# url-kaist/UV-SLAM

Measured on AMD Instinct MI355X. Metric: sliding-window solves/sec (10 KF, 150 pts, 40 lines, 3 VP), higher is better.
Workload: dtype f64; 1 GPU; W10-P150-L40-V3 x 256 independent windows per GPU (BASELINE configs[2]); single window (configs[1]) in single_window, the 20k-point window (configs[3]) in large_window (both with --full); windows_per_gpu=256, frames=11, points=150, lines=40, vp_tagged_lines=30, prior=True, parallelism=replicas x1

## Files before the change

uv-slam_amd/api.py:

```python
import ctypes as C
import os
import time

import numpy as np

from . import abi

_HERE = os.path.dirname(os.path.abspath(__file__))
LIB_PATH = os.environ.get("UVS_SOLVER_LIB", os.path.join(_HERE, "libuvs_solver.so"))
_lib = None

EXPORTS = [
    "uvs_abi_version", "uvs_default_options", "uvs_create", "uvs_destroy", "uvs_last_error", "uvs_status_string",
    "uvs_solve_window", "uvs_batch_upload", "uvs_batch_solve", "uvs_batch_download", "uvs_batch_stream", "uvs_evaluate", "uvs_marginalize", "uvs_marginalize_resident", "uvs_marginalize_batch",
    "uvs_reduced_dim", "uvs_pg_create", "uvs_pg_destroy", "uvs_pg_last_error", "uvs_pg_optimize", "uvs_pg_debug_step",
    "uvs_lc_create", "uvs_lc_destroy", "uvs_lc_last_error", "uvs_lc_verify", "uvs_lc_debug_pair",
    "uvs_vp_create", "uvs_vp_destroy", "uvs_vp_last_error", "uvs_vp_estimate", "uvs_vp_last_device_ms", "uvs_vp_debug_frame",
    "uvs_kf_create", "uvs_kf_destroy", "uvs_kf_last_error", "uvs_kf_extract", "uvs_kf_last_device_ms", "uvs_kf_debug_frame",
    "uvs_ft_create", "uvs_ft_destroy", "uvs_ft_last_error", "uvs_ft_reset", "uvs_ft_track", "uvs_ft_last_device_ms", "uvs_ft_debug_pyramid", "uvs_ft_debug_point",
    "uvs_ft_set_max_candidates", "uvs_ft_set_mask", "uvs_ft_detect", "uvs_ft_last_detect_device_ms", "uvs_ft_debug_detect",
    "uvs_ft_reject", "uvs_ft_last_reject_device_ms", "uvs_ft_debug_reject",
    "uvs_ft_set_equalize", "uvs_ft_equalize", "uvs_ft_last_equalize_device_ms", "uvs_ft_debug_equalize",
    "uvs_lt_create", "uvs_lt_destroy", "uvs_lt_last_error", "uvs_lt_reset", "uvs_lt_track", "uvs_lt_match", "uvs_lt_last_device_ms", "uvs_lt_debug_line",
    "uvs_lt_gauss_tables",
# ... 453 lines not shown
        try:
            for s, rc in zip(solvers, rcs): s._check(rc)

            def exchange(which, n):
                bufs = [np.zeros(n) for _ in solvers]
                for s, b in zip(solvers, bufs): s._check(L.uvs_large_exchange_host(s._h, which, abi._dp(b), 0))
                tot = bufs[0].copy()
                for b in bufs[1:]: tot = tot + b
                if which == 0: tot[n - 7] = max(b[n - 7] for b in bufs)
                for s in solvers: s._check(L.uvs_large_exchange_host(s._h, which, abi._dp(tot), 1))

            n = C.c_int(0)
            L.uvs_large_reduced(solvers[0]._h, C.byref(n)); n_red = n.value
            L.uvs_large_scalars(solvers[0]._h, C.byref(n)); n_sc = n.value
            for k in range(len(r)):
                for s in solvers:
                    assert L.uvs_large_need_linearize(s._h)
                    s._check(L.uvs_large_linearize(s._h))
                exchange(0, n_red)
                for s in solvers: s._check(L.uvs_large_step(s._h))
                exchange(1, n_sc)
                for s, (step, scal) in zip(solvers, out):
                    s._check(L.uvs_large_debug_step(s._h, float(r[k + 1]) if k + 1 < len(r) else 0.0, step.shape[1], abi._dp(step[k]), abi._dp(scal[k])))
        finally:
            for s in solvers:
                L.uvs_large_set_debug_step(s._h, 0); L.uvs_large_set_nranks(s._h, 1)
        return out

    def debug_first_iteration(self, w: abi.Window):
        wc, keep = w.to_c()
        S = np.zeros((176, 176)); g = np.zeros(176); hd = np.zeros(176); dd = np.zeros(176); step = np.zeros(176); scal = np.zeros(40)
        self._check(lib().uvs_debug_first_iteration(self._h, C.byref(wc), *[abi._dp(a) for a in (S, g, hd, dd, step, scal)]))
        return dict(S=S, g=g, hd=hd, dd=dd, step=step, cost=scal[0], gmax=scal[1], chol_ok=scal[2], mcc=scal[3], step2=scal[4],
                    cycles=dict(zip(['setup', 'obs', 'lmprep', 'gather', 'assemble', 'chol', 'trsv', 'backsub', 'cost', 'misc', 'chol_diag', 'chol_panel', 'chol_trail', 'asm_imu', 'asm_zero', 'asm_add'], scal[8:24])), sub_timers=dict(cost_phase=dict(zip(['stage_dx', 'prior_residual', 'observations', 'imu'], scal[24:28])), chol_busy_per_wave=scal[28:32].copy()))


class PoseGraphSolver(_Handle):

    _UNIT = "uvs_pg"

    def __init__(self, device=0, max_keyframes=16384, max_loops=256):
        self._create(device, max_keyframes, max_loops)

    def optimize_raw(self, t, q, sequence, constant, loops):
        p, keep = abi.pg_problem(t, q, sequence, constant, loops)
        out = np.zeros((max(p.n, 1), 4))
        rep = abi.PgReport()
        t0 = time.perf_counter()
        rc = lib().uvs_pg_optimize(self._h, C.byref(p), abi._dp(out), C.byref(rep))
        self.last_ms = (time.perf_counter() - t0) * 1e3
        return rc, out[:p.n], rep

    def optimize(self, t, q, sequence, constant, loops):
        rc, out, rep = self.optimize_raw(t, q, sequence, constant, loops)
        if rc not in (abi.UVS_OK, abi.UVS_ERR_NUMERIC):
            raise self._error("uvs_pg_optimize", rc)
        return out, rep

    def debug_step_raw(self, t, q, sequence, constant, loops, radius):
        p, keep = abi.pg_problem(t, q, sequence, constant, loops)
        delta = np.zeros(max(4 * int(np.count_nonzero(keep["constant"] == 0)), 1)); scal = np.zeros(abi.PG_DEBUG_SCAL_LEN)
        rc = lib().uvs_pg_debug_step(self._h, C.byref(p), float(radius), abi._dp(delta), abi._dp(scal))
        return rc, delta[:4 * int(scal[3])], scal

    def debug_step(self, t, q, sequence, constant, loops, radius):
        rc, delta, scal = self.debug_step_raw(t, q, sequence, constant, loops, radius)
# ... 886 lines not shown
```

uv-slam_amd/csrc/uvs_layout.h:

```cpp
#pragma once
#include <stdint.h>

#define UVS_NF 11
#define UVS_FD 16
#define UVS_RD (UVS_NF * UVS_FD)
#define UVS_NBLK (UVS_NF * (UVS_NF + 1) / 2)
#define UVS_NBLKX (UVS_NBLK + UVS_NF + 1 + UVS_NF + 2)
#define UVS_EX_INDEX(a) (16 * (a) + 15)
#define UVS_RELO_FRAME (UVS_NF + 1)
#define UVS_RELO2_BLOCKROW (UVS_NF + 2)
#define UVS_NBLKX2 (UVS_NBLKX + UVS_NF + 3)
#define UVS_RELO2_DOUBLES 2304
#define UVS_XDIM 192
#define UVS_TD_INDEX (UVS_RD - 1)
#define UVS_BLK_LD 17
#define UVS_BLK_SZ (16 * UVS_BLK_LD)
#define UVS_S_DOUBLES (UVS_NBLK * UVS_BLK_SZ)

#define UVS_IMU_STRIDE 296
#define UVS_IMU_JAC 20
#define UVS_IMU_COV 68
#define UVS_IMU_WS 226
#define UVS_IMU_JIDX(R, C, i, j) (9 * ((R) == 0 ? ((C) == 9 ? 0 : 1) : (R) == 3 ? 2 : ((C) == 9 ? 3 : 4)) + 3 * (i) + (j))

// ... 52 lines not shown
    int32_t d_lnmeas;
    int32_t d_imu;
    int32_t d_prior;
    int32_t i_pt_lm, i_pt_fi, i_pt_fj, i_pt_beg;
    int32_t i_ln_lm, i_ln_fj, i_ln_vp, i_ln_beg;
    int32_t i_imu;
    int32_t i_prior;
    int32_t i_chunks;
    int32_t i_wblk;
    int32_t i_lists;
    int32_t w_invd0, w_invd1, w_line0, w_line1;
    int32_t w_ltrig0, w_ltrig1;
    int32_t w_scale_pt, w_scale_ln;
    int32_t w_pt_E, w_pt_x;
    int32_t w_ln_Y, w_ln_x;
    int32_t w_imu;
    int32_t w_imu_w;
    int32_t w_out;
    int32_t w_prior_h0;
    int32_t n_pblk;
    int32_t w_gacc;
    int32_t n_cimg, w_cimg;
    int32_t ws_doubles;
    int32_t blob_bytes;
    int32_t cur_sel;
    int32_t max_chunk_doubles;
    int32_t n_parts;
    int32_t chol_half_ok;
    int32_t reserved0;
    int64_t out_host;
    int32_t redamp_ok;
};

#define UVS_PH_G0(n) ((((n) * (n)) + 1) & ~1)
#define UVS_PH_C0(n) (UVS_PH_G0(n) + UVS_MAX_PRIOR_DIM)
#define UVS_PH_HD(n) (UVS_PH_C0(n) + 8)
#define UVS_PH_DOUBLES(n) (UVS_PH_HD(n) + UVS_RD)
#define UVS_WIMU_STRIDE 936
#define UVS_LN_X 24
```

uv-slam_amd/csrc/uvs_solve_kernel.h:

```cpp
#pragma once
#include <hip/hip_runtime.h>
#include <initializer_list>
#include <utility>
#include "../../include/uvs_solver.h"
#include "uvs_layout.h"
#include "uvs_factors.h"

namespace uvsdev {

#ifndef UVS_UNIT
#define UVS_UNIT unit
#endif

#ifndef UVS_X_PLAIN_TID
static __device__ __forceinline__ int lane_tid() { int t = threadIdx.x; asm volatile("" : "+v"(t)); return t; }
#else
static __device__ __forceinline__ int lane_tid() { return threadIdx.x; }
#endif
static constexpr int NT = UVS_NT;
static constexpr int NW = NT / 64;
static constexpr bool ROLES = NT > 256;
static constexpr int ET = ROLES ? 256 : NT;
static constexpr int EW = ET / 64;
static constexpr int GT0 = NT - UVS_GT;
// ... 33 lines not shown
static constexpr int L_PRC = L_PR + UVS_MAX_PRIOR_DIM;
static constexpr int L_RED = L_PRC + UVS_MAX_PRIOR_DIM;
static constexpr int L_CTRL = L_RED + (5 * NW > 24 ? 5 * NW : 24);
static constexpr int L_PROF = L_CTRL + 32;
static constexpr int L_WPROF = L_PROF + 24;
static constexpr int L_LCOST = L_WPROF + 8;
static constexpr int LACC = 1;
static constexpr int L_LGMAX = L_LCOST + ET / LACC;
static constexpr int L_PX0 = L_LGMAX + 8;
static constexpr int L_PTAB = L_PX0 + 9 * UVS_MAX_PRIOR_BLOCKS;
static constexpr int L_SMALL = (L_PTAB + 2 * UVS_MAX_PRIOR_BLOCKS + 1) & ~1;
static constexpr int L_S = L_SMALL;
static constexpr int L_TOTAL = L_S + UVS_S_DOUBLES;
static_assert(L_TOTAL * 8 <= 160 * 1024, "LDS map exceeds the 160 KB of a CU");
enum { P_SETUP = 0, P_OBS, P_LMPREP, P_GATHER, P_ASSEMBLE, P_CHOL, P_TRSV, P_BACKSUB, P_COST, P_MISC, P_CH_DIAG, P_CH_PANEL, P_CH_TRAIL, P_AS_IMU, P_AS_ZERO, P_AS_ADD, P_LAST };
#define UVS_PROF(c, k) do { if ((c).o.debug && lane_tid() == 0) { const long long now_ = clock64(); (c).sh[L_PROF + (k)] += (double)(now_ - (long long)(c).sh[L_PROF + 23]); (c).sh[L_PROF + 23] = (double)now_; } } while (0)
static constexpr size_t LDS_BYTES = (size_t)L_TOTAL * 8;
static constexpr int TL_PER_WAVE = 4096;
inline namespace UVS_UNIT { __device__ long long g_lin_tl[8 * TL_PER_WAVE * 2]; }
#define UVS_TLOG(c, id) do { if ((c).o.debug == 5 && (threadIdx.x & 63) == 0 && blockIdx.x == 0) { const int w_ = threadIdx.x >> 6; const int n_ = (int)(c).sh[L_WPROF + w_]; \
    if (n_ < TL_PER_WAVE) { g_lin_tl[2 * (w_ * TL_PER_WAVE + n_)] = (id); g_lin_tl[2 * (w_ * TL_PER_WAVE + n_) + 1] = clock64(); (c).sh[L_WPROF + w_] = (double)(n_ + 1); } } } while (0)

enum { C_COST = 0, C_RADIUS, C_DECR, C_XNORM, C_GMAX, C_CAND, C_MCC, C_STEP2, C_XC2, C_GO, C_IT, C_INVALID, C_CUR, C_FIRST,
       C_TERM, C_NSUCC, C_CHOLOK, C_GMAXLM, C_TIMEUP };

struct KOpts {
    int max_it, ex_free, keep_cand, jacobi;
    double sqrt_info, line_factor, vp_factor, loss_pt, loss_ln, loss_vp, G[3];
    double r0, rmax, rmin, min_rel, dlo, dhi, ftol, gtol, ptol;
    int max_invalid;
    int debug;
    long long max_ticks;
    int redamp;
};

inline namespace UVS_UNIT {
__constant__ unsigned char c_blk_fa[UVS_NBLK];
__constant__ unsigned char c_blk_fb[UVS_NBLK];
}

UVS_DEV int sidx(int i, int j) {
    const int bi = i >> 4, bj = j >> 4;
    return (((bi * (bi + 1)) >> 1) + bj) * UVS_BLK_SZ + (i & 15) * UVS_BLK_LD + (j & 15);
}
UVS_DEV double bcast_lane(double v, int lane) {
    const int lo = __builtin_amdgcn_readlane(__double2loint(v), lane);
    const int hi = __builtin_amdgcn_readlane(__double2hiint(v), lane);
    return __hiloint2double(hi, lo);
}
UVS_DEV void wave_sync() {
    __builtin_amdgcn_fence(__ATOMIC_RELEASE, "wavefront");
    __builtin_amdgcn_wave_barrier();
    __builtin_amdgcn_fence(__ATOMIC_ACQUIRE, "wavefront");
}

UVS_DEV double wave_sum(double v) {
#pragma unroll
    for (int off = 32; off > 0; off >>= 1) v += __shfl_down(v, off, 64);
    return v;
}
UVS_DEV double wave_max(double v) {
#pragma unroll
    for (int off = 32; off > 0; off >>= 1) v = fmax(v, __shfl_down(v, off, 64));
    return v;
}
UVS_DEV void rsqrt_pair(double x, double* sq, double* rsq) {
// ... 984 lines not shown
#pragma unroll
                        for (int r = 0; r < GR; ++r) A.g[r] -= (ok && diag) ? o.gg[u][r] : 0.0;
                    }
                }
            });
    }
    if (DELTA) return;
    {
        struct Ops { double p0[GR], p1[GR]; d2_t q0[3], q1[3], rc; };
        const int e0 = on ? lists[UVS_NGRP + 1 + g] : 0, e1 = on ? lists[UVS_NGRP + 2 + g] : 0;
        gather_walk<1, Ops>(ent, e0, e1,
            [&](int, const int* w, Ops& o) {
                const int lo = w[0] & 0x7fff;
                const double* pa = S0 + lo + r0;
                const double* pb = S0 + ((unsigned)w[0] >> 16);
#pragma unroll
                for (int r = 0; r < GR; ++r) { o.p0[r] = pa[r]; o.p1[r] = pa[p1off + r]; }
#pragma unroll
                for (int k = 0; k < 3; ++k) { o.q0[k] = lds2(pb + 2 * k); o.q1[k] = lds2(pb + 6 + 2 * k); }
                o.rc = lds2(S0 + lo + ((w[0] & UVS_PT_ENTRY_A) ? UVS_PT_RC2 - UVS_PT_A : rcoff));
            },
            [&](int, Ops& o) {
#pragma unroll
                for (int r = 0; r < GR; ++r) {
                    if (dirv) { row_fma(A.v + 6 * r, o.p0[r], o.q0); row_fma(A.v + 6 * r, o.p1[r], o.q1); }
                    if (tdcol) A.v[6 * r] += o.p0[r] * o.q0[0].x + o.p1[r] * o.q0[0].y;
                    if (diag) { A.g[r] += o.p0[r] * o.rc.x + o.p1[r] * o.rc.y; A.hd[r] += o.p0[r] * o.p0[r] + o.p1[r] * o.p1[r]; }
                }
            });
    }
}

template <bool DELTA = false>
UVS_DEV void gather_lines(int grp, const int* lists, const double* S0, GAcc& A, int goff = 0, int eoff = 0) {
    const int g = (lane_tid() - GT0) / UVS_GLANES, r0 = GR * (lane_tid() % UVS_GLANES);
    const bool on = grp >= 0;
    const bool diag = on && ((grp >> 8) & 1);
    const int* ent = lists + LIST_HDR;
    {
        struct Ops { double ea[4][GR]; d2_t y[4][3]; double gg[DELTA ? GR : 1]; };
        const int e0 = on ? lists[g] : 0, e1 = on ? lists[g + 1] : 0;
        gather_walk<1, Ops>(ent, e0, e1,
            [&](int, const int* w, Ops& o) {
                const int lo = w[0] & 0x7fff;
                const double* pa = S0 + lo + r0;
                const double* pb = S0 + ((unsigned)w[0] >> 16);
#pragma unroll
                for (int q = 0; q < 4; ++q) {
#pragma unroll
                    for (int r = 0; r < GR; ++r) o.ea[q][r] = pa[6 * q + r];
                    o.y[q][0] = lds2(pb + 6 * q); o.y[q][1] = lds2(pb + 6 * q + 2); o.y[q][2] = lds2(pb + 6 * q + 4);
                }
                if (DELTA) {
                    const double* pg = S0 + goff + 6 * ((lo - eoff) / UVS_LN_EY) + r0;
#pragma unroll
                    for (int r = 0; r < GR; ++r) o.gg[r] = pg[r];
                }
            },
            [&](int, Ops& o) {
#pragma unroll
                for (int q = 0; q < 4; ++q)
#pragma unroll
                    for (int r = 0; r < GR; ++r) row_fma(A.v + 6 * r, -o.ea[q][r], o.y[q]);
                if (DELTA) {
#pragma unroll
                    for (int r = 0; r < GR; ++r) A.g[r] -= diag ? o.gg[r] : 0.0;
                }
            });
    }
    if (DELTA) return;
    {
        struct Ops { double p[3][GR]; d2_t q[3][3], rc01; double rc2; };
        const int e0 = on ? lists[UVS_NGRP + 1 + g] : 0, e1 = on ? lists[UVS_NGRP + 2 + g] : 0;
        gather_walk<1, Ops>(ent, e0, e1,
            [&](int, const int* w, Ops& o) {
                const double* R = S0 + w[0];
#pragma unroll
                for (int k = 0; k < 3; ++k) {
#pragma unroll
                    for (int r = 0; r < GR; ++r) o.p[k][r] = R[UVS_LN_JP + 6 * k + r0 + r];
                    o.q[k][0] = lds2(R + UVS_LN_JP + 6 * k); o.q[k][1] = lds2(R + UVS_LN_JP + 6 * k + 2); o.q[k][2] = lds2(R + UVS_LN_JP + 6 * k + 4);
                }
                o.rc01 = lds2(R); o.rc2 = R[UVS_LN_RV];
            },
            [&](int, Ops& o) {
#pragma unroll
                for (int r = 0; r < GR; ++r) {
#pragma unroll
                    for (int k = 0; k < 3; ++k) { row_fma(A.v + 6 * r, o.p[k][r], o.q[k]); A.hd[r] += o.p[k][r] * o.p[k][r]; }
                    A.g[r] += o.p[0][r] * o.rc01.x + o.p[1][r] * o.rc01.y + o.p[2][r] * o.rc2;
                }
            });
    }
}

static constexpr int IMU_JLD = 48;
static constexpr int IMU_WOFF = 16 * IMU_JLD;
static constexpr int IMU_BLK = IMU_WOFF + UVS_BLK_SZ;
#ifndef UVS_IMU_SLOT_SWAP
#define UVS_IMU_SLOT_SWAP 1
#endif
static constexpr int IMU_SLOTS = (UVS_NF - 1 + NW - 1) / NW;
UVS_DEV int imu_block_of(int wv, int s) {
    if (NW == 8 && UVS_IMU_SLOT_SWAP) return s == 0 ? wv : (wv == 0 ? 9 : wv == 1 ? 8 : UVS_NF);
    return wv + s * NW;
}
struct ImuN { d4_t n00[IMU_SLOTS], n10[IMU_SLOTS], n11[IMU_SLOTS]; int fi[IMU_SLOTS]; bool act[IMU_SLOTS]; };

UVS_DEV double lin_prep(const Ctx& c, const double* x, int mode = 0) {
// ... 278 lines not shown
        iacc += c.bi[h.i_pt_beg + lm] + c.bi[h.i_pt_beg + lm + 1];
    } else {
        const int lm = c.bi[h.i_ln_lm + o]; iacc = c.bi[h.i_ln_fj + o] + c.bi[h.i_ln_vp + o];
#ifndef UVS_X_NO_TOUCH_B1
        iacc += c.bi[h.i_ln_beg + lm] + c.bi[h.i_ln_beg + lm + 1];
        acc += c.ws[h.w_scale_ln + 4 * lm] + c.ws[h.w_scale_ln + 4 * lm + 3];
#endif
        const double* m = c.bd + h.d_lnmeas + o; const int st = h.ln_stride;
#pragma unroll
        for (int q = 0; q < 9; ++q) acc += m[q * st];
        const double* ltrig = line_trig_of(c, line);
        if (ltrig) {
#pragma unroll
            for (int q = 0; q < 8; ++q) acc += ltrig[8 * lm + q];
        } else {
#pragma unroll
            for (int q = 0; q < 4; ++q) acc += line[4 * lm + q];
        }
    }
    asm volatile("" :: "v"(acc), "v"(iacc));
}
static constexpr int LG_UN = 16;
UVS_DEV void copy_lists_gatherers(const Ctx& c, const ChunkDesc& d) {
    int* lists = chunk_lists(c, d);
    const int t0 = lane_tid() - GT0;
    for (int tb = t0; tb < d.nlist; tb += LG_UN * UVS_GT) {
        int w[LG_UN];
#pragma unroll
        for (int u = 0; u < LG_UN; ++u) { const int t = tb + u * UVS_GT; w[u] = d.glists[t < d.nlist ? t : tb]; }
#pragma unroll
        for (int u = 0; u < LG_UN; ++u) { const int t = tb + u * UVS_GT; if (t < d.nlist) lists[t] = w[u]; }
    }
}
UVS_DEV void chunk_eval(const Ctx& c, const ChunkDesc& d, const double* x, const double* invd, const double* line, bool first, double radius) {
    DevWinK& h = *c.hdr;
    double* sh = c.sh;
    const int tid = lane_tid();
    const double* RF = sh + L_RF; const double* ric = sh + L_EX; const double* tic = sh + L_EX + 9;
    double cost = 0.0, gmax_lm = 0.0;
    {
        const int type = d.type, k0 = d.k0, k1 = d.k1;
        const int* glists = d.glists;
        const int nlist = d.nlist;
        const int nlm = d.nlm;
        UVS_TLOG(c, 1);
        __syncthreads();
        UVS_PROF(c, P_GATHER);
        UVS_TLOG(c, 2);
        if (type == 0) {
            const int* beg = c.bi + h.i_pt_beg;
            const int o0 = d.o0, nob = d.nob, o1 = o0 + nob;
            const int PREC = h.pt_rec, XS = h.pt_xslots;
            double* rec = sh + L_S;
            double* Eb = rec + (size_t)nob * PREC;
            double* EIb = Eb + (size_t)(nob + XS * nlm) * 6;
            int* lists = (int*)(EIb + (size_t)(nob + XS * nlm) * 6);
            if (!LISTS_BY_GATHERERS) for (int t = tid; t < nlist; t += ET) lists[t] = glists[t];
            for (int o = o0 + tid; o < o1; o += ET) {
                const int lm = c.bi[h.i_pt_lm + o], fi = c.bi[h.i_pt_fi + o], fj = c.bi[h.i_pt_fj + o];
                double pi[3], pj[3], vij[4] = {0.0, 0.0, 0.0, 0.0};
                load_point_obs(c, o, x[183], pi, pj, vij);
                double r[2], A[12], B[12], cl[2], jtd[2] = {0.0, 0.0};
                point_eval<true, false>(x + 7 * fi, RF + 9 * fi, pose_of(x, fj), RF + 9 * fj, ric, tic, invd[lm], pi, pj, c.o.sqrt_info, r, A, B, cl, nullptr,
                                        vij, vij + 2, h.td_on ? jtd : nullptr);
                double sc; cost += 0.5 * cauchy(c.o.loss_pt, r[0] * r[0] + r[1] * r[1], &sc);
                double* R = rec + (size_t)(o - o0) * PREC;
// ... 10 lines not shown
                }
            }
            UVS_TLOG(c, 3);
            __syncthreads();
            UVS_PROF(c, P_OBS);
            UVS_TLOG(c, 4);
            for (int ol = tid; ol < nob; ol += ET) {
                const int k = c.bi[h.i_pt_lm + o0 + ol], li = k - k0, b0 = beg[k] - o0, b1 = beg[k + 1] - o0;
                double hd, gl; pt_landmark_hd_gl(rec, PREC, b0, b1, &hd, &gl);
                const bool lead = ol == b0;
                double sc;
                if (first) { sc = c.o.jacobi ? 1.0 / (1.0 + sqrt(hd)) : 1.0; if (lead && !ANCHOR_BY_GATHERERS) c.ws[h.w_scale_pt + k] = sc; } else sc = c.ws[h.w_scale_pt + k];
                const double dd = fmin(fmax(sc * sc * hd, c.o.dlo), c.o.dhi) / (radius * sc * sc);
                const double hinv = 1.0 / (hd + dd), ginv = gl * hinv;
                const int s = ol - b0 + 1;
                double* E = Eb + (size_t)(b0 + XS * li) * 6; double* EI = EIb + (size_t)(b0 + XS * li) * 6;
                double* Eg = c.ws + h.w_pt_E + 6 * (size_t)(o0 + b0 + XS * k);
                double* R = rec + (size_t)ol * PREC;
                const double c0 = R[UVS_PT_C], c1 = R[UVS_PT_C + 1], rr0 = R[0], rr1 = R[1];
                double Bv[12];
#pragma unroll
                for (int a = 0; a < 12; ++a) Bv[a] = R[UVS_PT_B + a];
#pragma unroll
                for (int a = 0; a < 6; ++a) { const double e = c0 * Bv[a] + c1 * Bv[6 + a]; E[6 * s + a] = e; EI[6 * s + a] = e * hinv; Eg[6 * s + a] = e * hinv; }
                R[UVS_PT_RC2] = rr0 - c0 * ginv; R[UVS_PT_RC2 + 1] = rr1 - c1 * ginv;
                if (lead && !ANCHOR_BY_GATHERERS) pt_landmark_slots(c, d, k, b0, b1, hd, gl, dd, hinv, ginv, &gmax_lm);
            }
            UVS_TLOG(c, 5);
            __syncthreads();
            UVS_PROF(c, P_LMPREP);
            UVS_TLOG(c, 7);
            lacc_add(sh, cost, gmax_lm);
        } else {
            const int* beg = c.bi + h.i_ln_beg;
            const int o0 = d.o0, nob = d.nob, o1 = o0 + nob;
            double* rec = sh + L_S;
            double* Eb = rec + (size_t)nob * UVS_LN_REC;
            double* Yb = Eb + (size_t)nob * UVS_LN_EY;
            double* Xb = Yb + (size_t)nob * UVS_LN_EY;
            int* lists = (int*)(Xb + 20 * nlm);
            if (!LISTS_BY_GATHERERS) for (int t = tid; t < nlist; t += ET) lists[t] = glists[t];
            const double* ltrig = line_trig_of(c, line);
            for (int o = o0 + tid; o < o1; o += ET) {
                const int lm = c.bi[h.i_ln_lm + o], fj = c.bi[h.i_ln_fj + o], hv = c.bi[h.i_ln_vp + o];
                const double* m = c.bd + h.d_lnmeas + o; const int st = h.ln_stride;
                const double sp[3] = {m[0], m[st], m[2 * st]}, ep[3] = {m[3 * st], m[4 * st], m[5 * st]}, vp[3] = {m[6 * st], m[7 * st], m[8 * st]};
                LineGeom g;
                line_geom<true>(x + 7 * fj, x + 7 * fj + 3, RF + 9 * fj, ric, tic, line + 4 * lm, g, ltrig ? ltrig + 8 * lm : nullptr);
                double* R = rec + (size_t)(o - o0) * UVS_LN_REC;
                double r[2], Jp[12], Jl[8], sc;
                line_residual<true>(g, sp, ep, c.o.line_factor, r, Jp, Jl);
                cost += 0.5 * cauchy(c.o.loss_ln, r[0] * r[0] + r[1] * r[1], &sc);
                R[0] = sc * r[0]; R[1] = sc * r[1];
#pragma unroll
                for (int q = 0; q < 12; ++q) R[UVS_LN_JP + q] = sc * Jp[q];
#pragma unroll
                for (int q = 0; q < 8; ++q) R[UVS_LN_JL + q] = sc * Jl[q];
                R[UVS_LN_RV + 1] = (double)((lm - k0) | (fj << 10));
                if (hv) {
                    double rv, Jvp[6], Jvl[4];
                    vp_residual<true>(g, vp, c.o.vp_factor, &rv, Jvp, Jvl);
                    cost += 0.5 * cauchy(c.o.loss_vp, rv * rv, &sc);
                    R[UVS_LN_RV] = sc * rv;
#pragma unroll
                    for (int q = 0; q < 6; ++q) R[UVS_LN_JP + 12 + q] = sc * Jvp[q];
#pragma unroll
                    for (int q = 0; q < 4; ++q) R[UVS_LN_JL + 8 + q] = sc * Jvl[q];
                } else {
#pragma unroll
                    for (int q = 0; q < 6; ++q) R[UVS_LN_JP + 12 + q] = 0.0;
                    R[UVS_LN_RV] = 0.0;
#pragma unroll
                    for (int q = 0; q < 4; ++q) R[UVS_LN_JL + 8 + q] = 0.0;
                }
            }
            UVS_TLOG(c, 3);
            __syncthreads();
            UVS_PROF(c, P_OBS);
            UVS_TLOG(c, 4);
            for (int li = tid; li < nlm; li += ET) {
                const int k = k0 + li, b0 = beg[k] - o0, b1 = beg[k + 1] - o0;
                double H[10] = {0, 0, 0, 0, 0, 0, 0, 0, 0, 0}, gl[4] = {0, 0, 0, 0};
                double scl[4] = {1.0, 1.0, 1.0, 1.0};
                if (!first) {
#pragma unroll
                    for (int a = 0; a < 4; ++a) scl[a] = c.ws[h.w_scale_ln + 4 * k + a];
                }
                for (int o = b0; o < b1; ++o) {
                    const double* R = rec + (size_t)o * UVS_LN_REC;
#pragma unroll
                    for (int a = 0; a < 4; ++a) {
                        gl[a] += R[UVS_LN_JL + a] * R[0] + R[UVS_LN_JL + 4 + a] * R[1] + R[UVS_LN_JL + 8 + a] * R[UVS_LN_RV];
#pragma unroll
                        for (int b = 0; b <= a; ++b) H[(a * (a + 1)) / 2 + b] += R[UVS_LN_JL + a] * R[UVS_LN_JL + b] + R[UVS_LN_JL + 4 + a] * R[UVS_LN_JL + 4 + b] + R[UVS_LN_JL + 8 + a] * R[UVS_LN_JL + 8 + b];
                    }
                }
                double* lx = c.ws + h.w_ln_x + UVS_LN_X * (size_t)k;
#pragma unroll
                for (int q = 0; q < 10; ++q) lx[12 + q] = H[q];
#pragma unroll
                for (int a = 0; a < 4; ++a) {
                    const double hd = H[(a * (a + 1)) / 2 + a];
                    double sc;
                    if (first) { sc = c.o.jacobi ? 1.0 / (1.0 + sqrt(hd)) : 1.0; c.ws[h.w_scale_ln + 4 * k + a] = sc; } else sc = scl[a];
                    const double dd = fmin(fmax(sc * sc * hd, c.o.dlo), c.o.dhi) / (radius * sc * sc);
                    H[(a * (a + 1)) / 2 + a] = hd + dd;
                    lx[4 + a] = gl[a]; lx[8 + a] = dd;
                    gmax_lm = fmax(gmax_lm, fabs(gl[a]));
                }
                double* X = Xb + 20 * li;
                double hg[4];
                spd4_inverse(H, gl, X, hg);
// ... 6 lines not shown
            for (int o = tid; o < nob; o += ET) {
                double* R = rec + (size_t)o * UVS_LN_REC;
                const int li = (int)R[UVS_LN_RV + 1] & 1023;
                double* E = Eb + (size_t)o * UVS_LN_EY; double* Y = Yb + (size_t)o * UVS_LN_EY;
                double* Yg = c.ws + h.w_ln_Y + 24 * (size_t)(o0 + o);
                double Xv[20], Jl[12], Jp[18];
#pragma unroll
                for (int q = 0; q < 20; ++q) Xv[q] = Xb[20 * li + q];
#pragma unroll
                for (int q = 0; q < 12; ++q) Jl[q] = R[UVS_LN_JL + q];
#pragma unroll
                for (int q = 0; q < 18; ++q) Jp[q] = R[UVS_LN_JP + q];
                const double rr0 = R[0], rr1 = R[1], rr2 = R[UVS_LN_RV];
#pragma unroll
                for (int a = 0; a < 6; ++a) {
                    double e[4];
#pragma unroll
                    for (int q = 0; q < 4; ++q) { e[q] = Jl[q] * Jp[a] + Jl[4 + q] * Jp[6 + a] + Jl[8 + q] * Jp[12 + a]; E[6 * q + a] = e[q]; }
#pragma unroll
                    for (int q = 0; q < 4; ++q) { const double y = Xv[4 * q] * e[0] + Xv[4 * q + 1] * e[1] + Xv[4 * q + 2] * e[2] + Xv[4 * q + 3] * e[3]; Y[6 * q + a] = y; Yg[6 * q + a] = y; }
                }
                R[0] = rr0 - (Jl[0] * Xv[16] + Jl[1] * Xv[17] + Jl[2] * Xv[18] + Jl[3] * Xv[19]);
                R[1] = rr1 - (Jl[4] * Xv[16] + Jl[5] * Xv[17] + Jl[6] * Xv[18] + Jl[7] * Xv[19]);
                R[UVS_LN_RV] = rr2 - (Jl[8] * Xv[16] + Jl[9] * Xv[17] + Jl[10] * Xv[18] + Jl[11] * Xv[19]);
            }
            __syncthreads();
            UVS_PROF(c, P_LMPREP);
            UVS_TLOG(c, 7);
            lacc_add(sh, cost, gmax_lm);
        }
    }
}
UVS_DEV int chunk_eval_barriers(const ChunkDesc& d) { return d.type == 0 ? 3 : 4; }
UVS_DEV void chunk_gather(const Ctx& c, const ChunkDesc& d, int grp, GAcc& acc) {
    DevWinK& h = *c.hdr;
    const double* rec = c.sh + L_S;
    const int* lists = chunk_lists(c, d);
    UVS_TLOG(c, 8);
    if (d.type == 0) {
        const long long tg0_ = clock64();
        if (h.td_on | h.ex_on) gather_points<true>(grp, lists, rec, acc, 0, h.ex_on != 0); else gather_points<false>(grp, lists, rec, acc);
        if (c.o.debug == 2 && (lane_tid() & 63) == 0) c.sh[L_WPROF + 4 + ((lane_tid() >> 6) & 3)] += (double)(clock64() - tg0_);
    } else gather_lines(grp, lists, rec, acc);
    UVS_TLOG(c, 10);
}
UVS_DEV void lin_chunk(const Ctx& c, int ch, const double* x, const double* invd, const double* line, bool first, double radius,
                       int grp, GAcc& acc) {
    const ChunkDesc d = chunk_desc(c, ch);
    chunk_eval(c, d, x, invd, line, first, radius);
    chunk_gather(c, d, grp, acc);
}

UVS_DEV int redamp_barriers(const ChunkDesc& d) { return d.type == 0 ? 2 : 3; }
UVS_DEV void redamp_prep(const Ctx& c, const ChunkDesc& d, double radius) {
    DevWinK& h = *c.hdr;
    double* sh = c.sh;
    const int tid = lane_tid();
    const int type = d.type, k0 = d.k0;
    const int* glists = d.glists;
    const int nlist = d.nlist;
    const int nlm = d.nlm;
    __syncthreads();
    double* rec = sh + L_S;
    if (type == 0) {
        const int* beg = c.bi + h.i_pt_beg;
        const int o0 = d.o0, nob = d.nob;
        const int PREC = h.pt_rec, XS = h.pt_xslots;
        double* Gb = rec;
        double* Eb = rec + (size_t)nob * PREC;
        double* EIb = Eb + (size_t)(nob + XS * nlm) * 6;
        int* lists = (int*)(EIb + (size_t)(nob + XS * nlm) * 6);
        for (int t = tid; t < nlist; t += ET) lists[t] = glists[t];
        for (int t = tid; t < nlm + nob; t += ET) {
            const bool anchor = t < nlm;
            const int ol = anchor ? 0 : t - nlm;
            const int k = anchor ? k0 + t : c.bi[h.i_pt_lm + o0 + ol], li = k - k0;
// ... 429 lines not shown
        __syncthreads();
    }
    UVS_TZ(6)
#undef UVS_TZ
    UVS_PROF(c, P_AS_ZERO);
    if (mode != 2) {
        asm_imu(c, N);
    }
    if (mode != 2) asm_prior(c);
    __syncthreads();
    UVS_PROF(c, P_AS_ADD);
    if (mode == 1) return;
    asm_finish(c, x, first, radius, cost, gmax_lm, mode);
    UVS_PROF(c, P_ASSEMBLE);
}

static constexpr int ROLE_PARTS_OFF = (UVS_NF - 1) * IMU_BLK;
static_assert(ROLE_PARTS_OFF + (8 * GR + 1) * UVS_GT <= UVS_S_DOUBLES, "IMU staging + part sums exceed the S region");
UVS_DEV void role_barriers(int n) { for (int i = 0; i < n; ++i) __syncthreads(); }
UVS_DEV void gacc_store(const Ctx& c, const GAcc& A) {
    double* W = c.ws + c.hdr->w_gacc + (lane_tid() - GT0);
#pragma unroll
    for (int q = 0; q < 6 * GR; ++q) __builtin_nontemporal_store(A.v[q], W + q * UVS_GT);
#pragma unroll
    for (int q = 0; q < GR; ++q) { __builtin_nontemporal_store(A.g[q], W + (6 * GR + q) * UVS_GT); __builtin_nontemporal_store(A.hd[q], W + (7 * GR + q) * UVS_GT); }
}
UVS_DEV void gacc_load(const Ctx& c, GAcc& A) {
    const double* W = c.ws + c.hdr->w_gacc + (lane_tid() - GT0);
#pragma unroll
    for (int q = 0; q < 6 * GR; ++q) A.v[q] = W[q * UVS_GT];
#pragma unroll
    for (int q = 0; q < GR; ++q) { A.g[q] = W[(6 * GR + q) * UVS_GT]; A.hd[q] = W[(7 * GR + q) * UVS_GT]; }
}
UVS_DEV void linearize_roles(const Ctx& c, const double* x, const double* invd, const double* line, bool first, double radius, int prep_mode, bool redamp) {
    DevWinK& h = *c.hdr;
    const bool ev = role_eval();
    { const double pc = lin_prep(c, x, redamp ? 2 : prep_mode); if (!redamp) lacc_set(c.sh, pc, 0.0); }
    double ic = 0.0;
    UVS_TLOG(c, 20);
    PriorAdd pa;
    ImuN N;
    if (ev) {
        ChunkDesc d = chunk_desc(c, 0);
        for (int ch = 0; ch < h.n_chunks; ++ch) {
            if (redamp) redamp_prep(c, d, radius);
            else {
                chunk_eval(c, d, x, invd, line, first, radius);
            }
            if (ch + 1 < h.n_chunks) {
                d = chunk_desc(c, ch + 1);
#ifdef UVS_CHUNK_TOUCH
                if (!redamp) chunk_touch(c, d, invd, line);
#endif
            }
        }
        UVS_TLOG(c, 21);
        lin_imu_stage(c, x);
#ifndef UVS_X_NO_PRIOR_AHEAD
        asm_prior_load(c, pa);
#endif
        ic = lin_imu_tiles(c, N);
        UVS_TLOG(c, 22);
        __syncthreads();
        asm_zero(c);
        __syncthreads();
        UVS_TLOG(c, 23);
        __syncthreads();
        UVS_TLOG(c, 24);
        asm_imu(c, N);
        UVS_TLOG(c, 25);
    } else {
        const int grp = gather_group(c);
        GAcc A;
        if (redamp) gacc_load(c, A); else gacc_zero(A);
        ChunkDesc d = chunk_desc(c, 0);
        for (int ch = 0; ch < h.n_chunks; ++ch) {
            if (redamp) { role_barriers(redamp_barriers(d)); redamp_gather(c, d, grp, A); }
            else {
                __syncthreads();
                if (LISTS_BY_GATHERERS) copy_lists_gatherers(c, d);
                AnchorPre ap; ap.b0 = 0; ap.b1 = 0; ap.sc = 1.0;
                if (ANCHOR_BY_GATHERERS && d.type == 0) pt_anchor_pre(c, d, first, ap);
                __syncthreads();
                if (ANCHOR_BY_GATHERERS && d.type == 0) pt_anchor_pass(c, d, first, radius, ap);
                role_barriers(chunk_eval_barriers(d) - 2);
                chunk_gather(c, d, grp, A);
            }
            if (ch + 1 < h.n_chunks) d = chunk_desc(c, ch + 1);
        }
        __syncthreads();
        if (h.redamp_ok && c.o.redamp) gacc_store(c, A);
        GAcc& T = A;
        gacc_gather_parts(T, grp, c.sh + L_S + ROLE_PARTS_OFF);
#ifndef UVS_X_NO_PRIOR_AHEAD
        asm_prior_load(c, pa);
#endif
        ic = lin_imu_tiles(c, N);
        __syncthreads();
        asm_zero(c);
        __syncthreads();
        asm_part0(c, grp, T);
        __syncthreads();
        asm_imu(c, N);
    }
#ifndef UVS_X_NO_PRIOR_AHEAD
    asm_prior_add(c, pa);
#else
    asm_prior(c);
#endif
    __syncthreads();
    UVS_TLOG(c, 26);
    asm_finish(c, x, first && !redamp, radius, lacc_cost(c.sh) + ic, lacc_gmax(c.sh), 0);
    UVS_TLOG(c, 27);
}

UVS_DEV void linearize(const Ctx& c, const double* x, const double* invd, const double* line, bool first, double radius, int prep_mode, GAcc& A) {
    if (ROLES) { linearize_roles(c, x, invd, line, first, radius, prep_mode, false); return; }
    DevWinK& h = *c.hdr;
    const int grp = gather_group(c);
    gacc_zero(A);
    { const double pc = lin_prep(c, x, prep_mode); lacc_set(c.sh, pc, 0.0); }
    {
        ChunkDesc d = chunk_desc(c, 0);
        for (int ch = 0; ch < h.n_chunks; ++ch) {
            chunk_eval(c, d, x, invd, line, first, radius);
            chunk_gather(c, d, grp, A);
            if (ch + 1 < h.n_chunks) d = chunk_desc(c, ch + 1);
        }
    }
    ImuN N;
    const double ic = lin_imu(c, x, N);
    lin_assemble(c, x, first, radius, grp, A, N, lacc_cost(c.sh) + ic, lacc_gmax(c.sh));
}

UVS_DEV void relinearize_damping(const Ctx& c, const double* x, double radius, GAcc& A) {
    if (ROLES) { linearize_roles(c, x, nullptr, nullptr, false, radius, 2, true); return; }
    DevWinK& h = *c.hdr;
    const int grp = gather_group(c);
    (void)lin_prep(c, x, 2);
    {
        ChunkDesc d = chunk_desc(c, 0);
        for (int ch = 0; ch < h.n_chunks; ++ch) {
            redamp_prep(c, d, radius);
            redamp_gather(c, d, grp, A);
            if (ch + 1 < h.n_chunks) d = chunk_desc(c, ch + 1);
        }
    }
    ImuN N;
    const double ic = lin_imu(c, x, N);
// ... 471 lines not shown
        UVS_TLOG(c, 37);
        UVS_PROF(c, P_COST);
        double cand = s4[0];
        if (!isfinite(cand)) cand = 1.7976931348623157e308;
        const double step_norm = sqrt(step2);
        const double rel = (cost - cand) / mcc;
        const bool successful = rel > o.min_rel;
        if (tid == 0) { rep->candidate_cost[ti] = cand; rep->step_norm[ti] = step_norm; rep->relative_decrease[ti] = rel; rep->cost[ti] = cost; rep->radius[ti] = radius; rep->gradient_max_norm[ti] = gmax; }
        bool stop = false;
        if (step_norm <= o.ptol * (x_norm + o.ptol)) { term = UVS_TERM_PARAMETER_TOL; stop = true; }
        else if (fabs(cost - cand) <= o.ftol * cost) { term = UVS_TERM_FUNCTION_TOL; stop = true; }
        if (stop && !(o.keep_cand && successful)) break;
        if (successful) {
            __syncthreads();
            if (tid < UVS_XDIM) sh[L_X + tid] = sh[L_XC + tid];
            cur ^= 1; ++nsucc;
            x_norm = sqrt(xc2);
            { const double t3 = 2.0 * rel - 1.0; radius = radius / fmax(1.0 / 3.0, 1.0 - t3 * t3 * t3); }
            radius = fmin(o.rmax, radius);
            decr = 2.0;
            cost = cand;
            need_lin = true; pending = ti; prep_mode = 1;
            if (tid == 0) { rep->accepted[ti] = 1; rep->cost[ti] = cost; rep->radius[ti] = radius; }
            if (stop) break;
        } else {
            radius = radius / decr; decr *= 2.0; need_lin = true; prep_mode = 2;
            if (tid == 0) { rep->accepted[ti] = 0; rep->radius[ti] = radius; }
        }
    }
    __syncthreads();
    UVS_PROF(c, P_MISC);
    if (o.debug && dbg.scal && tid < P_LAST) dbg.scal[8 + tid] = sh[L_PROF + tid];
    if (o.debug && dbg.scal && tid < 8) dbg.scal[24 + tid] = sh[L_WPROF + tid];
    if (tid < UVS_XDIM) c.ws[h.w_out + tid] = sh[L_X + tid];
    for (int k = tid; k < h.n_points; k += NT) c.ws[h.w_out + UVS_XDIM + k] = invd[cur][k];
    for (int k = tid; k < 4 * h.n_lines; k += NT) c.ws[h.w_out + UVS_XDIM + h.n_points + k] = line[cur][k];
    if (h.out_host) {
        double* od = (double*)h.out_host;
        if (tid < UVS_XDIM) od[tid] = sh[L_X + tid];
        for (int k = tid; k < h.n_points; k += NT) od[UVS_XDIM + k] = invd[cur][k];
        for (int k = tid; k < 4 * h.n_lines; k += NT) od[UVS_XDIM + h.n_points + k] = line[cur][k];
    }
    if (tid == 0) {
        rep->status = status; rep->termination = term; rep->num_iterations = it; rep->num_successful = nsucc; rep->final_cost = cost;
        ((DevWin*)blob)->cur_sel = cur;
    }
}
#ifdef UVS_EMIT_K_SOLVE
__global__ __launch_bounds__(NT) void k_solve(char* blobs, const long long* blob_off, double* ws_all, const long long* ws_off,
                                              KOpts o, uvs_report* reports, DebugOut dbg) {
    extern __shared__ __attribute__((aligned(16))) double sh[];
    k_solve_body<false>(blobs, blob_off, ws_all, ws_off, o, reports, dbg, DebugStep{}, sh);
}
#endif
#ifdef UVS_EMIT_K_SOLVE_DSTEP
__global__ __launch_bounds__(NT) void k_solve_dstep(char* blobs, const long long* blob_off, double* ws_all, const long long* ws_off,
                                                    KOpts o, uvs_report* reports, DebugStep ds) {
    extern __shared__ __attribute__((aligned(16))) double sh[];
    DebugOut dbg; dbg.S = nullptr; dbg.g = nullptr; dbg.hd = nullptr; dbg.dd = nullptr; dbg.step = nullptr; dbg.scal = nullptr;
    k_solve_body<true>(blobs, blob_off, ws_all, ws_off, o, reports, dbg, ds, sh);
}
#endif

static int unit_init(const unsigned char* fa, const unsigned char* fb, int n, std::initializer_list<const void*> kernels) {
    if (n != UVS_NBLK) return UVS_ERR_INVALID_ARG;
    if (hipMemcpyToSymbol(HIP_SYMBOL(c_blk_fa), fa, n) != hipSuccess || hipMemcpyToSymbol(HIP_SYMBOL(c_blk_fb), fb, n) != hipSuccess) return UVS_ERR_HIP;
// ... 5 lines not shown
```

uv-slam_amd/csrc/uvs_solver_handle.h:

```cpp
#pragma once
#include <algorithm>
#include <chrono>
#include <condition_variable>
#include <cstdlib>
#include <functional>
#include <memory>
#include <mutex>
#include <pthread.h>
#include <sched.h>
#include <string>
#include <thread>
#include <vector>

#include "../../include/uvs_solver.h"
#include "uvs_hip_buf.h"
#include "uvs_layout.h"
#include "uvs_pack.h"
#include "uvs_solve_kernel.h"

#pragma GCC visibility push(hidden)

struct PackPool {
    std::vector<std::thread> th; std::mutex m; std::condition_variable cv_go, cv_done;
    const std::function<void(int)>* job = nullptr; int gen = 0, pending = 0; bool stop = false;
// ... 89 lines not shown
        bool active = false; int n_chunks = 0, sel = 0, it = 0, invalid = 0, nsucc = 0, pending = 0, term = 0, status = 0;
        bool need_lin = true, first = true, done = false;
        bool stored = false; int backsub_wgs = 0;
        double radius = 0, decr = 2, cost = 0, gmax = 0, x_norm = 0, local_x2 = 0;
        uvs_report rep;
        double frame_x2 = 0;
        double relo_pose_in[7] = {0, 0, 0, 0, 0, 0, 0};
        int grid = 0;
        std::chrono::steady_clock::time_point t_begin;
    } L;
    struct LargeBufs {
        DevBuf<double> d_state, d_partials, d_reduced, d_bsums, d_out, d_sc5;
        DevBuf<double> d_ctl; DevBuf<uvs_report> d_rep;
        DevBuf<double> d_fimg;
        void* comm = nullptr; int rank = 0, nranks = 1;
        int step_nranks = 1;
        bool debug_step = false; DevBuf<double> d_lstep;
    } LB;
    uvs_solver(); ~uvs_solver();
};

inline uvsdev::KOpts make_kopts(const uvs_options& o, int debug) {
    uvsdev::KOpts k;
    k.max_it = o.max_num_iterations; k.ex_free = o.estimate_extrinsic; k.keep_cand = o.function_tol_keeps_candidate; k.jacobi = o.jacobi_scaling;
    k.sqrt_info = o.point_sqrt_info; k.line_factor = o.line_factor; k.vp_factor = o.vp_factor;
    k.loss_pt = o.loss_point; k.loss_ln = o.loss_line; k.loss_vp = o.loss_vp;
    k.G[0] = o.gravity[0]; k.G[1] = o.gravity[1]; k.G[2] = o.gravity[2];
    k.r0 = o.initial_trust_region_radius; k.rmax = o.max_trust_region_radius; k.rmin = o.min_trust_region_radius;
    k.min_rel = o.min_relative_decrease; k.dlo = o.min_lm_diagonal; k.dhi = o.max_lm_diagonal;
    k.ftol = o.function_tolerance; k.gtol = o.gradient_tolerance; k.ptol = o.parameter_tolerance;
    k.max_ticks = o.max_solver_time_in_seconds > 0.0 ? std::max(1LL, (long long)(o.max_solver_time_in_seconds * 1e8)) : 0LL;
    k.max_invalid = o.max_consecutive_invalid_steps; k.debug = debug;
    { const char* e = std::getenv("UVS_REDAMP"); k.redamp = (e && e[0] == '0') ? 0 : 1; }
    return k;
}

inline PackPool& pack_pool(uvs_solver* s) { if (!s->pool) s->pool = std::make_shared<PackPool>(); return *s->pool; }

int upload_windows(uvs_solver* s, int n, const uvs_window* const* ws, bool wait, int chunk_grid = 0, bool out_direct = false, bool all_blocks = false);
int marg_unit_init(const unsigned char* fa, const unsigned char* fb, int n);
void marg_worker_release(uvs_solver* s);
int large_unit_init(const unsigned char* fa, const unsigned char* fb, int n);
int debug_step_large(uvs_solver* s, const uvs_window* w, int n_radii, const double* radii, int n_step, double* step, double* scal);
#pragma GCC visibility pop
```

Measured before the change: 192,500 solves/s.

## Run line-chunk residual pass ahead while gatherers consume previous chunk

In the role-split linearization, evaluator threads now compute the first pass of the next line chunk (residual and Jacobian records) into a spare region of shared memory while the gatherer threads are still accumulating the current chunk. Gatherers read line records at the matching offset, and the second pass runs later on the precomputed records. The aim is to hide the per-observation line evaluation behind the gather phase and shorten each chunk's critical path. It depends on free shared-memory space past the current chunk; when none is available it falls back to the old path. Adds an env toggle and debug counters.

```diff
diff --git a/uv-slam_amd/api.py b/uv-slam_amd/api.py
--- a/uv-slam_amd/api.py
+++ b/uv-slam_amd/api.py
@@ -509,6 +509,7 @@
         S = np.zeros((176, 176)); g = np.zeros(176); hd = np.zeros(176); dd = np.zeros(176); step = np.zeros(176); scal = np.zeros(40)
         self._check(lib().uvs_debug_first_iteration(self._h, C.byref(wc), *[abi._dp(a) for a in (S, g, hd, dd, step, scal)]))
         return dict(S=S, g=g, hd=hd, dd=dd, step=step, cost=scal[0], gmax=scal[1], chol_ok=scal[2], mcc=scal[3], step2=scal[4],
+                    line_ahead=int(scal[5]), linearizations=int(scal[6]),
                     cycles=dict(zip(['setup', 'obs', 'lmprep', 'gather', 'assemble', 'chol', 'trsv', 'backsub', 'cost', 'misc', 'chol_diag', 'chol_panel', 'chol_trail', 'asm_imu', 'asm_zero', 'asm_add'], scal[8:24])), sub_timers=dict(cost_phase=dict(zip(['stage_dx', 'prior_residual', 'observations', 'imu'], scal[24:28])), chol_busy_per_wave=scal[28:32].copy()))
 
 
diff --git a/uv-slam_amd/csrc/uvs_layout.h b/uv-slam_amd/csrc/uvs_layout.h
--- a/uv-slam_amd/csrc/uvs_layout.h
+++ b/uv-slam_amd/csrc/uvs_layout.h
@@ -108,6 +108,26 @@
     int32_t redamp_ok;
 };
 
+#if defined(__HIPCC__)
+#define UVS_LAYOUT_HD __host__ __device__ inline
+#else
+#define UVS_LAYOUT_HD inline
+#endif
+UVS_LAYOUT_HD int uvs_chunk_end(int type, int nob, int nlm, int nlist, int pt_rec, int pt_xslots) {
+    const int body = type == 0 ? nob * pt_rec + (nob + pt_xslots * nlm) * 12 : nob * (UVS_LN_REC + 2 * UVS_LN_EY) + 20 * nlm;
+    return body + (nlist + 1) / 2;
+}
+UVS_LAYOUT_HD int uvs_line_ahead_base(int cur_end, int cur_rec_base, int cur_rec_size, int next_type, int next_nob, int next_nlm, int next_nlist) {
+    if (next_type != 1 || next_nob <= 0) return -1;
+    const int nrec = next_nob * UVS_LN_REC;
+    if (cur_rec_base > 0 && nrec <= cur_rec_size && nrec <= cur_rec_base) return 0;
+    const int next_end = uvs_chunk_end(1, next_nob, next_nlm, next_nlist, 0, 0);
+    int hi = cur_end > next_end ? cur_end : next_end;
+    if (cur_rec_base + cur_rec_size > hi) hi = cur_rec_base + cur_rec_size;
+    hi = (hi + 1) & ~1;
+    return hi + nrec <= UVS_S_DOUBLES ? hi : -1;
+}
+
 #define UVS_PH_G0(n) ((((n) * (n)) + 1) & ~1)
 #define UVS_PH_C0(n) (UVS_PH_G0(n) + UVS_MAX_PRIOR_DIM)
 #define UVS_PH_HD(n) (UVS_PH_C0(n) + 8)
diff --git a/uv-slam_amd/csrc/uvs_solve_kernel.h b/uv-slam_amd/csrc/uvs_solve_kernel.h
--- a/uv-slam_amd/csrc/uvs_solve_kernel.h
+++ b/uv-slam_amd/csrc/uvs_solve_kernel.h
@@ -89,6 +89,7 @@
     int debug;
     long long max_ticks;
     int redamp;
+    int line_ahead;
 };
 
 inline namespace UVS_UNIT {
@@ -1139,7 +1140,7 @@
 }
 
 template <bool DELTA = false>
-UVS_DEV void gather_lines(int grp, const int* lists, const double* S0, GAcc& A, int goff = 0, int eoff = 0) {
+UVS_DEV void gather_lines(int grp, const int* lists, const double* S0, GAcc& A, int goff = 0, int eoff = 0, int roff = 0) {
     const int g = (lane_tid() - GT0) / UVS_GLANES, r0 = GR * (lane_tid() % UVS_GLANES);
     const bool on = grp >= 0;
     const bool diag = on && ((grp >> 8) & 1);
@@ -1181,7 +1182,7 @@
         const int e0 = on ? lists[UVS_NGRP + 1 + g] : 0, e1 = on ? lists[UVS_NGRP + 2 + g] : 0;
         gather_walk<1, Ops>(ent, e0, e1,
             [&](int, const int* w, Ops& o) {
-                const double* R = S0 + w[0];
+                const double* R = S0 + roff + w[0];
 #pragma unroll
                 for (int k = 0; k < 3; ++k) {
 #pragma unroll
@@ -1526,6 +1527,8 @@
         for (int u = 0; u < LG_UN; ++u) { const int t = tb + u * UVS_GT; if (t < d.nlist) lists[t] = w[u]; }
     }
 }
+UVS_DEV double line_pass_a(const Ctx& c, const ChunkDesc& d, const double* x, const double* line, int rec_base);
+UVS_DEV void line_pass_b(const Ctx& c, const ChunkDesc& d, bool first, double radius, double cost, int rec_base);
 UVS_DEV void chunk_eval(const Ctx& c, const ChunkDesc& d, const double* x, const double* invd, const double* line, bool first, double radius) {
     DevWinK& h = *c.hdr;
     double* sh = c.sh;
@@ -1602,14 +1605,25 @@
             UVS_TLOG(c, 7);
             lacc_add(sh, cost, gmax_lm);
         } else {
-            const int* beg = c.bi + h.i_ln_beg;
-            const int o0 = d.o0, nob = d.nob, o1 = o0 + nob;
-            double* rec = sh + L_S;
-            double* Eb = rec + (size_t)nob * UVS_LN_REC;
-            double* Yb = Eb + (size_t)nob * UVS_LN_EY;
-            double* Xb = Yb + (size_t)nob * UVS_LN_EY;
-            int* lists = (int*)(Xb + 20 * nlm);
-            if (!LISTS_BY_GATHERERS) for (int t = tid; t < nlist; t += ET) lists[t] = glists[t];
+            if (!LISTS_BY_GATHERERS) { int* lists = chunk_lists(c, d); for (int t = tid; t < nlist; t += ET) lists[t] = glists[t]; }
+            cost = line_pass_a(c, d, x, line, 0);
+            UVS_TLOG(c, 3);
+            __syncthreads();
+            UVS_PROF(c, P_OBS);
+            UVS_TLOG(c, 4);
+            line_pass_b(c, d, first, radius, cost, 0);
+        }
+    }
+}
+UVS_DEV double line_pass_a(const Ctx& c, const ChunkDesc& d, const double* x, const double* line, int rec_base) {
+    DevWinK& h = *c.hdr;
+    const int tid = lane_tid();
+    const double* RF = c.sh + L_RF; const double* ric = c.sh + L_EX; const double* tic = c.sh + L_EX + 9;
+    double cost = 0.0;
+    {
+        {
+            const int k0 = d.k0, o0 = d.o0, o1 = o0 + d.nob;
+            double* rec = c.sh + L_S + rec_base;
             const double* ltrig = line_trig_of(c, line);
             for (int o = o0 + tid; o < o1; o += ET) {
                 const int lm = c.bi[h.i_ln_lm + o], fj = c.bi[h.i_ln_fj + o], hv = c.bi[h.i_ln_vp + o];
@@ -1644,10 +1658,23 @@
                     for (int q = 0; q < 4; ++q) R[UVS_LN_JL + 8 + q] = 0.0;
                 }
             }
-            UVS_TLOG(c, 3);
-            __syncthreads();
-            UVS_PROF(c, P_OBS);
-            UVS_TLOG(c, 4);
+        }
+    }
+    return cost;
+}
+UVS_DEV void line_pass_b(const Ctx& c, const ChunkDesc& d, bool first, double radius, double cost, int rec_base) {
+    DevWinK& h = *c.hdr;
+    double* sh = c.sh;
+    const int tid = lane_tid();
+    double gmax_lm = 0.0;
+    {
+        {
+            const int* beg = c.bi + h.i_ln_beg;
+            const int k0 = d.k0, nlm = d.nlm, o0 = d.o0, nob = d.nob;
+            double* rec = sh + L_S + rec_base;
+            double* Eb = sh + L_S + (size_t)nob * UVS_LN_REC;
+            double* Yb = Eb + (size_t)nob * UVS_LN_EY;
+            double* Xb = Yb + (size_t)nob * UVS_LN_EY;
             for (int li = tid; li < nlm; li += ET) {
                 const int k = k0 + li, b0 = beg[k] - o0, b1 = beg[k + 1] - o0;
                 double H[10] = {0, 0, 0, 0, 0, 0, 0, 0, 0, 0}, gl[4] = {0, 0, 0, 0};
@@ -1720,7 +1747,7 @@
     }
 }
 UVS_DEV int chunk_eval_barriers(const ChunkDesc& d) { return d.type == 0 ? 3 : 4; }
-UVS_DEV void chunk_gather(const Ctx& c, const ChunkDesc& d, int grp, GAcc& acc) {
+UVS_DEV void chunk_gather(const Ctx& c, const ChunkDesc& d, int grp, GAcc& acc, int rec_base = 0) {
     DevWinK& h = *c.hdr;
     const double* rec = c.sh + L_S;
     const int* lists = chunk_lists(c, d);
@@ -1729,7 +1756,7 @@
         const long long tg0_ = clock64();
         if (h.td_on | h.ex_on) gather_points<true>(grp, lists, rec, acc, 0, h.ex_on != 0); else gather_points<false>(grp, lists, rec, acc);
         if (c.o.debug == 2 && (lane_tid() & 63) == 0) c.sh[L_WPROF + 4 + ((lane_tid() >> 6) & 3)] += (double)(clock64() - tg0_);
-    } else gather_lines(grp, lists, rec, acc);
+    } else gather_lines(grp, lists, rec, acc, 0, 0, rec_base);
     UVS_TLOG(c, 10);
 }
 UVS_DEV void lin_chunk(const Ctx& c, int ch, const double* x, const double* invd, const double* line, bool first, double radius,
@@ -2225,6 +2252,18 @@
 #pragma unroll
     for (int q = 0; q < GR; ++q) { A.g[q] = W[(6 * GR + q) * UVS_GT]; A.hd[q] = W[(7 * GR + q) * UVS_GT]; }
 }
+#ifndef UVS_X_NO_LINE_AHEAD
+static constexpr bool LINE_AHEAD = ROLES;
+#else
+static constexpr bool LINE_AHEAD = false;
+#endif
+static constexpr int DBG_N_LIN = 21, DBG_N_AHEAD = 22;
+UVS_DEV int line_ahead_base(const Ctx& c, const ChunkDesc& d, int rb, const ChunkDesc& dn) {
+    if (!LINE_AHEAD || !c.o.line_ahead || dn.type != 1) return -1;
+    DevWinK& h = *c.hdr;
+    const int rsz = d.nob * (d.type == 0 ? h.pt_rec : UVS_LN_REC);
+    return uvs_line_ahead_base(uvs_chunk_end(d.type, d.nob, d.nlm, d.nlist, h.pt_rec, h.pt_xslots), rb, rsz, dn.type, dn.nob, dn.nlm, dn.nlist);
+}
 UVS_DEV void linearize_roles(const Ctx& c, const double* x, const double* invd, const double* line, bool first, double radius, int prep_mode, bool redamp) {
     DevWinK& h = *c.hdr;
     const bool ev = role_eval();
@@ -2235,15 +2274,32 @@
     ImuN N;
     if (ev) {
         ChunkDesc d = chunk_desc(c, 0);
+        int rb = -1;
+        double acost = 0.0;
         for (int ch = 0; ch < h.n_chunks; ++ch) {
             if (redamp) redamp_prep(c, d, radius);
-            else {
+            else if (rb >= 0) {
+                UVS_TLOG(c, 1);
+                __syncthreads();
+                UVS_PROF(c, P_GATHER);
+                UVS_TLOG(c, 2);
+                line_pass_b(c, d, first, radius, acost, rb);
+                __syncthreads();
+            } else {
                 chunk_eval(c, d, x, invd, line, first, radius);
             }
             if (ch + 1 < h.n_chunks) {
-                d = chunk_desc(c, ch + 1);
+                const ChunkDesc dn = chunk_desc(c, ch + 1);
+                rb = redamp ? -1 : line_ahead_base(c, d, rb > 0 ? rb : 0, dn);
+                d = dn;
+                if (rb >= 0) {
+                    UVS_TLOG(c, 9);
+                    acost = line_pass_a(c, d, x, line, rb);
+                    UVS_TLOG(c, 3);
+                    if (c.o.debug && lane_tid() == 0) c.sh[L_PROF + DBG_N_AHEAD] += 1.0;
+                }
 #ifdef UVS_CHUNK_TOUCH
-                if (!redamp) chunk_touch(c, d, invd, line);
+                else if (!redamp) chunk_touch(c, d, invd, line);
 #endif
             }
         }
@@ -2267,6 +2323,7 @@
         GAcc A;
         if (redamp) gacc_load(c, A); else gacc_zero(A);
         ChunkDesc d = chunk_desc(c, 0);
+        int rb = 0;
         for (int ch = 0; ch < h.n_chunks; ++ch) {
             if (redamp) { role_barriers(redamp_barriers(d)); redamp_gather(c, d, grp, A); }
             else {
@@ -2277,9 +2334,14 @@
                 __syncthreads();
                 if (ANCHOR_BY_GATHERERS && d.type == 0) pt_anchor_pass(c, d, first, radius, ap);
                 role_barriers(chunk_eval_barriers(d) - 2);
-                chunk_gather(c, d, grp, A);
-            }
-            if (ch + 1 < h.n_chunks) d = chunk_desc(c, ch + 1);
+                chunk_gather(c, d, grp, A, rb);
+            }
+            if (ch + 1 < h.n_chunks) {
+                const ChunkDesc dn = chunk_desc(c, ch + 1);
+                const int nb = redamp ? -1 : line_ahead_base(c, d, rb, dn);
+                rb = nb > 0 ? nb : 0;
+                d = dn;
+            }
         }
         __syncthreads();
         if (h.redamp_ok && c.o.redamp) gacc_store(c, A);
@@ -2308,6 +2370,7 @@
 }
 
 UVS_DEV void linearize(const Ctx& c, const double* x, const double* invd, const double* line, bool first, double radius, int prep_mode, GAcc& A) {
+    if (c.o.debug && lane_tid() == 0) c.sh[L_PROF + DBG_N_LIN] += 1.0;
     if (ROLES) { linearize_roles(c, x, invd, line, first, radius, prep_mode, false); return; }
     DevWinK& h = *c.hdr;
     const int grp = gather_group(c);
@@ -2845,6 +2908,7 @@
     UVS_PROF(c, P_MISC);
     if (o.debug && dbg.scal && tid < P_LAST) dbg.scal[8 + tid] = sh[L_PROF + tid];
     if (o.debug && dbg.scal && tid < 8) dbg.scal[24 + tid] = sh[L_WPROF + tid];
+    if (o.debug && dbg.scal && tid == 0) { dbg.scal[5] = sh[L_PROF + DBG_N_AHEAD]; dbg.scal[6] = sh[L_PROF + DBG_N_LIN]; }
     if (tid < UVS_XDIM) c.ws[h.w_out + tid] = sh[L_X + tid];
     for (int k = tid; k < h.n_points; k += NT) c.ws[h.w_out + UVS_XDIM + k] = invd[cur][k];
     for (int k = tid; k < 4 * h.n_lines; k += NT) c.ws[h.w_out + UVS_XDIM + h.n_points + k] = line[cur][k];
diff --git a/uv-slam_amd/csrc/uvs_solver_handle.h b/uv-slam_amd/csrc/uvs_solver_handle.h
--- a/uv-slam_amd/csrc/uvs_solver_handle.h
+++ b/uv-slam_amd/csrc/uvs_solver_handle.h
@@ -145,6 +145,7 @@
     k.max_ticks = o.max_solver_time_in_seconds > 0.0 ? std::max(1LL, (long long)(o.max_solver_time_in_seconds * 1e8)) : 0LL;
     k.max_invalid = o.max_consecutive_invalid_steps; k.debug = debug;
     { const char* e = std::getenv("UVS_REDAMP"); k.redamp = (e && e[0] == '0') ? 0 : 1; }
+    { const char* e = std::getenv("UVS_LINE_AHEAD"); k.line_ahead = (e && e[0] == '0') ? 0 : 1; }
     return k;
 }
 
```

Measured after the change: 195,800 solves/s (median of 6 runs). 1.7% higher.
